# ilyakurdyukov/jpeg-quantsmooth

Hardware: AMD Instinct MI355X
Metric: 8x8 blocks/s at q=3 niter=3 (higher is better)
Workload: dtype f32

## Files before the change

### jpeg-quantsmooth_amd/csrc/qs_kernels.hip

```cpp
#include <hip/hip_runtime.h>
#include <stdint.h>
#include <stdlib.h>
#include "qs_device.h"
#include "qs_devfn.h"



__device__ __forceinline__ void wave_lds_sync() {
  __builtin_amdgcn_fence(__ATOMIC_RELEASE, "wavefront");
  __builtin_amdgcn_wave_barrier();
  __builtin_amdgcn_fence(__ATOMIC_ACQUIRE, "wavefront");
}

__device__ __forceinline__ uint32_t mulc(uint32_t a, int c) {
  return (uint32_t)__mul24((int)a, c);
}

__device__ __forceinline__ uint32_t lshl13_add(uint32_t x, uint32_t b) {
  uint32_t r;
  asm("v_lshl_add_u32 %0, %1, 13, %2" : "=v"(r) : "v"(x), "v"(b));
  return r;
}

__device__ __forceinline__ void idct8(uint32_t (&v)[8], uint32_t bias) {
  uint32_t z1, z2, z3, z4, z5, t0, t1, t2, t3, e0, e1, e2, e3;
  z2 = v[2]; z3 = v[6];
  z1 = mulc(z2 + z3, 4433);
  asm volatile("" : "+v"(z1));
  t2 = z1 - mulc(z3, 15137);
  t3 = z1 + mulc(z2, 6270);
  t0 = lshl13_add(v[0] + v[4], bias);
  t1 = lshl13_add(v[0] - v[4], bias);
  e0 = t0 + t3; e3 = t0 - t3; e1 = t1 + t2; e2 = t1 - t2;
  t0 = v[7]; t1 = v[5]; t2 = v[3]; t3 = v[1];
  z1 = t0 + t3; z2 = t1 + t2; z3 = t0 + t2; z4 = t1 + t3;
  z5 = mulc(z3 + z4, 9633);
  asm volatile("" : "+v"(z5));
  t0 = mulc(t0, 2446);  t1 = mulc(t1, 16819);
  t2 = mulc(t2, 25172); t3 = mulc(t3, 12299);
  z1 = mulc(z1, 7373);  z2 = mulc(z2, 20995);
  z3 = mulc(z3, 16069); z4 = mulc(z4, 3196);
  z3 = z5 - z3; z4 = z5 - z4;
  t0 += z3 - z1; t1 += z4 - z2; t2 += z3 - z2; t3 += z4 - z1;
  v[0] = e0 + t3; v[7] = e0 - t3;
  v[1] = e1 + t2; v[6] = e1 - t2;
  v[2] = e2 + t1; v[5] = e2 - t1;
  v[3] = e3 + t0; v[4] = e3 - t0;
}

__device__ __forceinline__ void idct_pass1(uint32_t (&ws)[64]) {
#pragma unroll
  for (int x = 0; x < 8; ++x) {
    uint32_t col[8];
#pragma unroll
    for (int j = 0; j < 8; ++j) col[j] = ws[j * 8 + x];
    idct8(col, 1024u);
#pragma unroll
    for (int j = 0; j < 8; ++j) ws[j * 8 + x] = (uint32_t)((int32_t)col[j] >> 11);
  }
}

__device__ __forceinline__ void idct_pass2_row(uint32_t (&row)[8], int (&out)[8]) {
  idct8(row, 257u << 17);
#pragma unroll
  for (int j = 0; j < 8; ++j) {
    int z = (int32_t)row[j];
    z = min(max(z, 0), (256 << 18) - 1);
    out[j] = z >> 18;
  }
}

#define QS_PIX_BITS 0x45000000u
__device__ __forceinline__ void idct_pass2_row_f(uint32_t (&row)[8], float (&out)[8]) {
  idct8(row, 257u << 17);
#pragma unroll
  for (int j = 0; j < 8; ++j) {
    int z = (int32_t)row[j];
    z = min(max(z, 0), (256 << 18) - 1);
    out[j] = __builtin_bit_cast(float, __builtin_amdgcn_alignbit(QS_PIX_BITS >> 14, (uint32_t)z, 18));
  }
}
__device__ __forceinline__ float pix_from_byte(uint32_t v, int n) {
  return __builtin_bit_cast(float, QS_PIX_BITS | ((v >> (8 * n)) & 0xffu));
}

__device__ __forceinline__ void
store_pixel_row(uint8_t* __restrict__ org, int pitch, int y, const int (&o)[8], int bx, int by, int wblk, int hblk,
                int rep_top, int rep_bot) {
  uint2 pk;
  pk.x = (uint32_t)o[0] | ((uint32_t)o[1] << 8) | ((uint32_t)o[2] << 16) | ((uint32_t)o[3] << 24);
  pk.y = (uint32_t)o[4] | ((uint32_t)o[5] << 8) | ((uint32_t)o[6] << 16) | ((uint32_t)o[7] << 24);
  uint8_t* rp = org + (size_t)y * pitch;
  *reinterpret_cast<uint2*>(rp) = pk;
  const bool top = (y == 0 && by == 0 && rep_top), bot = (y == 7 && by == hblk - 1 && rep_bot);
  if (bx == 0) {
    rp[-1] = (uint8_t)o[0];
    if (top) rp[-1 - pitch] = (uint8_t)o[0];
    if (bot) rp[-1 + pitch] = (uint8_t)o[0];
  }
  if (bx == wblk - 1) {
    rp[8] = (uint8_t)o[7];
    if (top) rp[8 - pitch] = (uint8_t)o[7];
    if (bot) rp[8 + pitch] = (uint8_t)o[7];
  }
  if (top) *reinterpret_cast<uint2*>(rp - pitch) = pk;
  if (bot) *reinterpret_cast<uint2*>(rp + pitch) = pk;
}

__device__ __forceinline__ void
idct_ws_to_plane(uint32_t (&ws)[64], uint8_t* __restrict__ plane, int wblk, int hblk, int pitch,
                 int rep_top, int rep_bot, int blk) {
  const int by = blk / wblk, bx = blk - by * wblk;
  idct_pass1(ws);
  uint8_t* org = plane + (size_t)(by * 8 + 1) * pitch + QS_APRON_X + bx * 8;
#pragma unroll
  for (int y = 0; y < 8; ++y) {
    uint32_t row[8]; int o[8];
#pragma unroll
    for (int j = 0; j < 8; ++j) row[j] = ws[y * 8 + j];
    idct_pass2_row(row, o);
    store_pixel_row(org, pitch, y, o, bx, by, wblk, hblk, rep_top, rep_bot);
  }
}

__device__ __forceinline__ void
idct_wave_to_plane(const QsConsts* __restrict__ cst, int16_t* __restrict__ coef,
                   uint8_t* __restrict__ plane, int wblk, int hblk, int pitch,
                   int first, int defer, int rep_top, int rep_bot, int* __restrict__ status, int base, uint32_t* lds) {
  const int lane = threadIdx.x & 63;
  const int nblk = wblk * hblk;
  const int nvec = min(64, nblk - base) * 8;
  uint4* gsrc = reinterpret_cast<uint4*>(coef) + (size_t)base * 8;
  uint4 v[8];
#pragma unroll
  for (int j = 0; j < 8; ++j) {
    const int idx = j * 64 + lane;
    v[j] = make_uint4(0, 0, 0, 0);
    if (idx < nvec) v[j] = gsrc[idx];
  }
  if (first) {
    int q[8], bad = 0;
    qs_load_qraw8(cst, lane & 7, q);
#pragma unroll
    for (int j = 0; j < 8; ++j) v[j] = qs_dequant8<true>(v[j], q, bad);
    if (!defer) {
#pragma unroll
      for (int j = 0; j < 8; ++j) {
        const int idx = j * 64 + lane;
        if (idx < nvec) gsrc[idx] = v[j];
      }
    }
    if (bad) atomicOr(status, 1);
  }
  {
    const int m0 = (lane & 7) * 4;
#pragma unroll
    for (int j = 0; j < 8; ++j) {
      uint32_t* dst = lds + m0 * QS_LDS_PITCH + (j * 8 + (lane >> 3));
      dst[0] = v[j].x; dst[QS_LDS_PITCH] = v[j].y; dst[2 * QS_LDS_PITCH] = v[j].z; dst[3 * QS_LDS_PITCH] = v[j].w;
    }
  }
  wave_lds_sync();
  const uint32_t* col = lds + lane;
  uint32_t ws[64];
#pragma unroll
  for (int r = 0; r < 32; ++r) {
    const uint32_t d = col[r * QS_LDS_PITCH];
    ws[r * 2] = (uint32_t)(int32_t)(int16_t)(d & 0xffff);
    ws[r * 2 + 1] = (uint32_t)((int32_t)d >> 16);
  }
  if (base + lane < nblk) idct_ws_to_plane(ws, plane, wblk, hblk, pitch, rep_top, rep_bot, base + lane);
}

__global__ void __launch_bounds__(256)
qs_idct_plane_kernel(const QsConsts* __restrict__ cst, int16_t* __restrict__ coef,
                     uint8_t* __restrict__ plane, int wblk, int hblk, int pitch,
                     int first, int rep_top, int rep_bot, int* __restrict__ status) {
  __shared__ uint32_t lds_all[4][32 * QS_LDS_PITCH];
  const int wave = threadIdx.x >> 6;
  const int base = __builtin_amdgcn_readfirstlane((int)(blockIdx.x * 256 + wave * 64));
  if (base >= wblk * hblk) return;
  idct_wave_to_plane(cst, coef, plane, wblk, hblk, pitch, first & 1, first & 2, rep_top, rep_bot, status, base, lds_all[wave]);
}

__global__ void __launch_bounds__(256)
qs_idct_set_kernel(const QsPlaneSet set, int first) {
  __shared__ uint32_t lds_all[4][32 * QS_LDS_PITCH];
  const int wave = threadIdx.x >> 6;
  const int w = __builtin_amdgcn_readfirstlane((int)(blockIdx.x * 4 + wave));
  if (w >= set.wave0[set.n]) return;
  const int i = qs_set_find(set, w);
  const QsPlaneRef& r = set.ref[i];
  const int base = (w - set.wave0[i]) * 64;
  if (base >= r.wblk * r.hblk) return;
  idct_wave_to_plane(r.cst, r.coef, r.plane, r.wblk, r.hblk, r.pitch, first, r.mode & QS_PLANE_QUANT,
                     r.mode & QS_PLANE_REP_TOP, r.mode & QS_PLANE_REP_BOT, r.status, base, lds_all[wave]);
}



typedef int16_t __attribute__((may_alias)) lds_i16;
__device__ __forceinline__ int lds_coef(const uint32_t* col, int i) {
  const lds_i16* p = reinterpret_cast<const lds_i16*>(col + (i >> 1) * QS_LDS_PITCH) + (i & 1);
  return *p;
}
__device__ __forceinline__ void lds_set_coef(uint32_t* col, int i, int v) {
  lds_i16* p = reinterpret_cast<lds_i16*>(col + (i >> 1) * QS_LDS_PITCH) + (i & 1);
  *p = (lds_i16)v;
}

static_assert(QS_LDS_PITCH * 4 == 260, "the literal offsets below assume a 260-byte row pitch");
#define QS_LDS16_GROUP(BASE, W, N0, O) \
  asm volatile("ds_read_i16 %0, %16 offset:" #O "\n\tds_read_i16 %1, %16 offset:" #O "+2\n\t" \
               "ds_read_i16 %2, %16 offset:" #O "+260\n\tds_read_i16 %3, %16 offset:" #O "+262\n\t" \
               "ds_read_i16 %4, %16 offset:" #O "+520\n\tds_read_i16 %5, %16 offset:" #O "+522\n\t" \
               "ds_read_i16 %6, %16 offset:" #O "+780\n\tds_read_i16 %7, %16 offset:" #O "+782\n\t" \
               "ds_read_i16 %8, %16 offset:" #O "+1040\n\tds_read_i16 %9, %16 offset:" #O "+1042\n\t" \
               "ds_read_i16 %10, %16 offset:" #O "+1300\n\tds_read_i16 %11, %16 offset:" #O "+1302\n\t" \
               "ds_read_i16 %12, %16 offset:" #O "+1560\n\tds_read_i16 %13, %16 offset:" #O "+1562\n\t" \
               "ds_read_i16 %14, %16 offset:" #O "+1820\n\tds_read_i16 %15, %16 offset:" #O "+1822\n\t" \
               "s_waitcnt lgkmcnt(0)" \
               : "=&v"(W[(N0) + 0]), "=&v"(W[(N0) + 1]), "=&v"(W[(N0) + 2]), "=&v"(W[(N0) + 3]), \
                 "=&v"(W[(N0) + 4]), "=&v"(W[(N0) + 5]), "=&v"(W[(N0) + 6]), "=&v"(W[(N0) + 7]), \
                 "=&v"(W[(N0) + 8]), "=&v"(W[(N0) + 9]), "=&v"(W[(N0) + 10]), "=&v"(W[(N0) + 11]), \
                 "=&v"(W[(N0) + 12]), "=&v"(W[(N0) + 13]), "=&v"(W[(N0) + 14]), "=&v"(W[(N0) + 15]) \
               : "v"(BASE) : "memory")
__device__ __forceinline__ void lds_read_block_i16(const uint32_t* col, uint32_t (&ws)[64]) {
  typedef const __attribute__((address_space(3))) uint32_t* lds_ptr;
  const uint32_t a0 = (uint32_t)(uintptr_t)(lds_ptr)col;
  const uint32_t a1 = a0 + 8 * 260, a2 = a0 + 16 * 260, a3 = a0 + 24 * 260;
  QS_LDS16_GROUP(a0, ws, 0, 0);
  QS_LDS16_GROUP(a1, ws, 16, 0);
  QS_LDS16_GROUP(a2, ws, 32, 0);
  QS_LDS16_GROUP(a3, ws, 48, 0);
}
__device__ __forceinline__ void lds_read_block_i16_1(const uint32_t* col, uint32_t (&ws)[64]) {
  typedef const __attribute__((address_space(3))) uint32_t* lds_ptr;
  const uint32_t a0 = (uint32_t)(uintptr_t)(lds_ptr)col;
  QS_LDS16_GROUP(a0, ws, 0, 0);
  QS_LDS16_GROUP(a0, ws, 16, 2080);
  QS_LDS16_GROUP(a0, ws, 32, 4160);
  QS_LDS16_GROUP(a0, ws, 48, 6240);
}

#define QS_PIX_SCALE 0.000244140625f
#define QS_TERM_D(D, W) { \
    float u_ = __builtin_amdgcn_fmed3f(Rs - __builtin_fabsf(D), 0.0f, 1.0f); \
    float t_ = u_ * u_; \
    float x_ = (D) * t_; \
    float y_ = (W) * t_; \
    num = num + x_ * y_; \
    den = den + y_ * y_; }
#define QS_TERM(A, B, W) { float d_ = (A) - (B); QS_TERM_D(d_, W) }

typedef float qs_w16 __attribute__((ext_vector_type(16)));
typedef int qs_i4 __attribute__((ext_vector_type(4)));
#define QS_SWAIT(BUF) asm volatile("s_waitcnt lgkmcnt(0)" : "+s"(BUF) : : "memory")

#define QS_WAVES_PER_WG 4
#define QS_SMOOTH_MIN_WAVES 3
#define QS_RESIDENT_WG (256 * QS_SMOOTH_MIN_WAVES * 4 / QS_WAVES_PER_WG)
#define QS_PRIO_SLOW 3
#define QS_PRIO_TERMS 0

#define QS_TERM_OPT(COND, A, B, W) { float d_, t_; \
        asm volatile( \
          "s_cmp_lg_u32 %[c], 0\n\t" \
          "s_cbranch_scc1 1f\n\t" \
          "v_sub_f32 %[d], %[a], %[b]\n\t" \
          "v_sub_f32 %[t], %[r], |%[d]| clamp\n\t" \
          "v_mul_f32 %[t], %[t], %[t]\n\t" \
          "v_mul_f32 %[d], %[d], %[t]\n\t" \
          "v_mul_f32 %[t], %[w], %[t]\n\t" \
          "v_mul_f32 %[d], %[d], %[t]\n\t" \
          "v_add_f32 %[n], %[n], %[d]\n\t" \
          "v_mul_f32 %[d], %[t], %[t]\n\t" \
          "v_add_f32 %[e], %[e], %[d]\n" \
          "1:" \
          : [n] "+v"(num), [e] "+v"(den), [d] "=&v"(d_), [t] "=&v"(t_) \
          : [a] "v"(A), [b] "v"(B), [w] "s"(W), [r] "s"(Rs), [c] "s"(COND) : "scc"); }
#define QS_TERM_ASM(A, B, W) { float d_, t_; \
        asm volatile( \
          "v_sub_f32 %[d], %[a], %[b]\n\t" \
          "v_sub_f32 %[t], %[r], |%[d]| clamp\n\t" \
          "v_mul_f32 %[t], %[t], %[t]\n\t" \
          "v_mul_f32 %[d], %[d], %[t]\n\t" \
          "v_mul_f32 %[t], %[w], %[t]\n\t" \
          "v_mul_f32 %[d], %[d], %[t]\n\t" \
          "v_add_f32 %[n], %[n], %[d]\n\t" \
          "v_mul_f32 %[d], %[t], %[t]\n\t" \
          "v_add_f32 %[e], %[e], %[d]" \
          : [n] "+v"(num), [e] "+v"(den), [d] "=&v"(d_), [t] "=&v"(t_) \
          : [a] "v"(A), [b] "v"(B), [w] "s"(W), [r] "s"(Rs)); }

#define QS_TERM_D_ASM(D, W) { float d_, t_; \
        asm volatile( \
          "v_sub_f32 %[t], %[r], |%[a]| clamp\n\t" \
          "v_mul_f32 %[t], %[t], %[t]\n\t" \
          "v_mul_f32 %[d], %[a], %[t]\n\t" \
          "v_mul_f32 %[t], %[w], %[t]\n\t" \
          "v_mul_f32 %[d], %[d], %[t]\n\t" \
          "v_add_f32 %[n], %[n], %[d]\n\t" \
          "v_mul_f32 %[d], %[t], %[t]\n\t" \
          "v_add_f32 %[e], %[e], %[d]" \
          : [n] "+v"(num), [e] "+v"(den), [d] "=&v"(d_), [t] "=&v"(t_) \
          : [a] "v"(D), [w] "s"(W), [r] "s"(Rs)); }
#ifndef QS_HOIST_DIAG
#define QS_HOIST_DIAG 32
#endif
#ifndef QS_Q1_SKIP
#define QS_Q1_SKIP 1
#endif
#ifndef QS_STASH
#define QS_STASH 1
#endif
#define QS_X_STASH 0
#define QS_X_EDGE 8
#define QS_X_REB 16
#define QS_X_DWORDS 20
static_assert(QS_WAVES_PER_WG * (32 * QS_LDS_PITCH + QS_X_DWORDS * 64) * 4 <= 160 * 1024 / 3, "LDS budget of three workgroups per CU");
typedef unsigned long long __attribute__((address_space(3))) qs_lds_u64;
__device__ __forceinline__ void qs_lds_add64(qs_lds_u64* p, long long v) {
  __hip_atomic_fetch_add(p, (unsigned long long)v, __ATOMIC_RELAXED, __HIP_MEMORY_SCOPE_WAVEFRONT);
}
__device__ __forceinline__ qs_lds_u64* qs_xreb(const uint32_t* col, const uint32_t* lds, int n) {
  typedef const __attribute__((address_space(3))) uint32_t* lds_ptr;
  uint32_t a = (uint32_t)(uintptr_t)(lds_ptr)col;
  asm volatile("" : "+v"(a));
  const uint32_t b = (uint32_t)(uintptr_t)(lds_ptr)lds;
  return (qs_lds_u64*)(a * 2u - b + (uint32_t)((32 * QS_LDS_PITCH + (QS_X_REB + 2 * n) * 64) * 4));
}

#define QS_SMOOTH_KERNEL_NAME qs_smooth_plane_kernel
#include "qs_smooth_kernel.inc"
#undef QS_SMOOTH_KERNEL_NAME
#define QS_SMOOTH_KERNEL_NAME qs_smooth_set_kernel
#define QS_SMOOTH_SET 1
#include "qs_smooth_kernel.inc"
#undef QS_SMOOTH_KERNEL_NAME
#undef QS_SMOOTH_SET

#define QS_DP_KERNEL_NAME qs_smooth_dp_kernel
#include "qs_smooth_dp_kernel.inc"
#undef QS_DP_KERNEL_NAME
#define QS_DP_KERNEL_NAME qs_smooth_dp_set_kernel
#define QS_DP_SET 1
#include "qs_smooth_dp_kernel.inc"
#undef QS_DP_KERNEL_NAME
#undef QS_DP_SET

__global__ void __launch_bounds__(256)
qs_clamp_kernel(int16_t* __restrict__ coef, size_t nvec) {
  size_t i = (size_t)blockIdx.x * 256 + threadIdx.x;
  const size_t stride = (size_t)gridDim.x * 256;
  uint4* p = reinterpret_cast<uint4*>(coef);
  for (; i < nvec; i += stride) {
    uint4 v = p[i];
    uint32_t d[4] = {v.x, v.y, v.z, v.w};
#pragma unroll
    for (int c = 0; c < 4; ++c) {
      int lo = (int16_t)(d[c] & 0xffff), hi = (int32_t)d[c] >> 16;
      lo = min(max(lo, -1023), 1023); hi = min(max(hi, -1023), 1023);
      d[c] = ((uint32_t)lo & 0xffffu) | ((uint32_t)hi << 16);
    }
    p[i] = make_uint4(d[0], d[1], d[2], d[3]);
  }
}

__global__ void __launch_bounds__(256)
qs_dequant_kernel(const QsConsts* __restrict__ cst, int16_t* __restrict__ coef, size_t nvec) {
  size_t i = (size_t)blockIdx.x * 256 + threadIdx.x;
  const size_t stride = (size_t)gridDim.x * 256;
  uint4* p = reinterpret_cast<uint4*>(coef);
  for (; i < nvec; i += stride) {
    uint4 v = p[i];
    uint32_t d[4] = {v.x, v.y, v.z, v.w};
    const int j = (int)(i & 7);
#pragma unroll
    for (int c = 0; c < 4; ++c) {
      int lo = (int16_t)(d[c] & 0xffff), hi = (int32_t)d[c] >> 16;
      lo *= cst->qraw[j * 8 + c * 2]; hi *= cst->qraw[j * 8 + c * 2 + 1];
      d[c] = ((uint32_t)lo & 0xffffu) | ((uint32_t)hi << 16);
    }
    p[i] = make_uint4(d[0], d[1], d[2], d[3]);
  }
}

#include "qs_launch.h"

void qs_launch_idct_plane(const QsConsts* cst, int16_t* coef, uint8_t* plane, int wblk, int hblk,
                          int first, int rep_top, int rep_bot, int* status, hipStream_t s) {
  const int nblk = wblk * hblk;
  const int f = first == 3 ? 3 : first ? 1 : 0;
  hipLaunchKernelGGL(qs_idct_plane_kernel, dim3((nblk + 255) / 256), dim3(256), 0, s,
                     cst, coef, plane, wblk, hblk, qs_plane_pitch(wblk), f, rep_top, rep_bot, status);
}

#define QS_DP_WAVES 4
static int qs_dp_waves(int groups) {
  static const int on = [] { const char* v = getenv("QS_HIP_DP"); return v ? atoi(v) : 1; }();
  static const int lim = [] { const char* v = getenv("QS_HIP_DP_GROUPS"); return v ? atoi(v) : 768; }();
  static const int lim2 = [] { const char* v = getenv("QS_HIP_DP_GROUPS2"); return v ? atoi(v) : 1536; }();
  if (!on) return 0;
  return groups <= lim ? QS_DP_WAVES : groups <= lim2 ? 2 : 0;
}

void qs_launch_smooth_plane(const QsConsts* cst, int16_t* coef, const uint8_t* plane, uint8_t* plane_next, int rep_top, int rep_bot,
                            int wblk, int hblk, int diag, int rebalance, int final_clamp, int blk_begin, int blk_end, hipStream_t s) {
  const int n = blk_end - blk_begin;
  if (n <= 0) return;
  const int pitch = qs_plane_pitch(wblk);
  const int rep = (rep_top ? QS_PLANE_REP_TOP : 0) | (rep_bot ? QS_PLANE_REP_BOT : 0);
  if (const int nw = qs_dp_waves((n + 63) / 64)) {
    const dim3 g((n + 63) / 64), b(64 * nw);
#define QS_GO_DP(D, W) hipLaunchKernelGGL((qs_smooth_dp_kernel<D, W>), g, b, 0, s, cst, coef, plane, plane_next, rep, wblk, hblk, pitch, rebalance, final_clamp, blk_begin, blk_end)
    if (nw == 2) { if (diag) QS_GO_DP(true, 2); else QS_GO_DP(false, 2); }
    else if (diag) QS_GO_DP(true, QS_DP_WAVES); else QS_GO_DP(false, QS_DP_WAVES);
#undef QS_GO_DP
    return;
  }
  const int per_wg = 64 * QS_WAVES_PER_WG;
  const dim3 grid((n + per_wg - 1) / per_wg), block(per_wg);
#define QS_GO(K) hipLaunchKernelGGL(K, grid, block, 0, s, cst, coef, plane, plane_next, rep, wblk, hblk, pitch, rebalance, final_clamp, blk_begin, blk_end)
  if (diag) QS_GO(qs_smooth_plane_kernel<true>); else QS_GO(qs_smooth_plane_kernel<false>);
#undef QS_GO
}

void qs_launch_idct_set(const QsPlaneSet& set, int first, hipStream_t s) {
  const int nw = set.wave0[set.n];
  if (nw <= 0) return;
  hipLaunchKernelGGL(qs_idct_set_kernel, dim3((nw + 3) / 4), dim3(256), 0, s, set, first);
}

void qs_launch_smooth_set(const QsPlaneSet& set, int diag, int final_clamp, hipStream_t s) {
  const int nw = set.wave0[set.n];
  if (nw <= 0) return;
  if (const int dw = qs_dp_waves(nw)) {
    const dim3 g(nw), b(64 * dw);
#define QS_GO_DP(D, W) hipLaunchKernelGGL((qs_smooth_dp_set_kernel<D, W>), g, b, 0, s, set, final_clamp)
    if (dw == 2) { if (diag) QS_GO_DP(true, 2); else QS_GO_DP(false, 2); }
    else if (diag) QS_GO_DP(true, QS_DP_WAVES); else QS_GO_DP(false, QS_DP_WAVES);
#undef QS_GO_DP
    return;
  }
  const dim3 grid((nw + QS_WAVES_PER_WG - 1) / QS_WAVES_PER_WG), block(64 * QS_WAVES_PER_WG);
  if (diag) hipLaunchKernelGGL(qs_smooth_set_kernel<true>, grid, block, 0, s, set, final_clamp);
  else      hipLaunchKernelGGL(qs_smooth_set_kernel<false>, grid, block, 0, s, set, final_clamp);
}

void qs_launch_clamp(int16_t* coef, size_t nblk, hipStream_t s) {
  const size_t nvec = nblk * 8;
  const int grid = (int)((nvec + 255) / 256 < 8192 ? (nvec + 255) / 256 : 8192);
  hipLaunchKernelGGL(qs_clamp_kernel, dim3(grid ? grid : 1), dim3(256), 0, s, coef, nvec);
}

void qs_launch_dequant(const QsConsts* cst, int16_t* coef, size_t nblk, hipStream_t s) {
  const size_t nvec = nblk * 8;
  const int grid = (int)((nvec + 255) / 256 < 8192 ? (nvec + 255) / 256 : 8192);
  hipLaunchKernelGGL(qs_dequant_kernel, dim3(grid ? grid : 1), dim3(256), 0, s, cst, coef, nvec);
}
```

### jpeg-quantsmooth_amd/csrc/qs_smooth_kernel.inc

```
template <bool DIAG>
__global__ void __launch_bounds__(64 * QS_WAVES_PER_WG, QS_SMOOTH_MIN_WAVES)
#ifdef QS_SMOOTH_SET
QS_SMOOTH_KERNEL_NAME(const QsPlaneSet set, int final_clamp) {
  __shared__ __attribute__((aligned(16))) uint32_t lds_all[QS_WAVES_PER_WG][32 * QS_LDS_PITCH + (DIAG ? 0 : QS_X_DWORDS * 64)];
#if QS_STASH
  __shared__ uint32_t stash_all[QS_WAVES_PER_WG][2 * 8 * 64];
#endif
  const int lane = threadIdx.x & 63, wave = DIAG ? (int)(threadIdx.x >> 6) : __builtin_amdgcn_readfirstlane((int)(threadIdx.x >> 6));
  uint32_t* lds = lds_all[wave];
  uint32_t* col = lds + lane;
  const int gw = __builtin_amdgcn_readfirstlane((int)(blockIdx.x * QS_WAVES_PER_WG + wave));
  if (gw >= set.wave0[set.n]) return;
  const int pi = qs_set_find(set, gw);
  const QsConsts* __restrict__ cst = set.ref[pi].cst;
  int16_t* __restrict__ coef = set.ref[pi].coef;
  const uint8_t* __restrict__ plane = set.ref[pi].plane;
  const int wblk = set.ref[pi].wblk, hblk = set.ref[pi].hblk, pitch = set.ref[pi].pitch;
  const int rebalance = set.ref[pi].mode & QS_PLANE_REBALANCE;
  const int nblk = wblk * hblk;
  const int base = (gw - set.wave0[pi]) * 64;
  (void)hblk;
#else
QS_SMOOTH_KERNEL_NAME(const QsConsts* __restrict__ cst, int16_t* __restrict__ coef,
                       const uint8_t* __restrict__ plane, uint8_t* __restrict__ plane_next, int rep,
                       int wblk, int hblk, int pitch,
                       int rebalance, int final_clamp, int blk_begin, int blk_end) {
  __shared__ __attribute__((aligned(16))) uint32_t lds_all[QS_WAVES_PER_WG][32 * QS_LDS_PITCH + (DIAG ? 0 : QS_X_DWORDS * 64)];
#if QS_STASH
  __shared__ uint32_t stash_all[QS_WAVES_PER_WG][2 * 8 * 64];
#endif
  const int lane = threadIdx.x & 63, wave = DIAG ? (int)(threadIdx.x >> 6) : __builtin_amdgcn_readfirstlane((int)(threadIdx.x >> 6));
  uint32_t* lds = lds_all[wave];
  uint32_t* col = lds + lane;
  const int nblk = blk_end;
  const int base = blk_begin + (blockIdx.x * QS_WAVES_PER_WG + wave) * 64;
#endif
  if (base >= nblk) return;
  const int tail_prio = __builtin_amdgcn_readfirstlane(
      (gridDim.x > QS_RESIDENT_WG && blockIdx.x >= (gridDim.x / QS_RESIDENT_WG) * QS_RESIDENT_WG) ? 1 : 0);
  const int nvec = min(64, nblk - base) * 8;
#ifdef QS_STAGGER
  { unsigned hwid; asm volatile("s_getreg_b32 %0, hwreg(HW_REG_HW_ID)" : "=s"(hwid)); if (hwid & 1u) __builtin_amdgcn_s_sleep(QS_STAGGER); }
#endif

  uint4* gsrc = reinterpret_cast<uint4*>(coef) + (size_t)base * 8;
  uint32_t bigacc = 0;
#define QS_BIG_ACC(V) if constexpr (!DIAG) bigacc |= ((V).x ^ ((V).x << 1)) | ((V).y ^ ((V).y << 1)) | ((V).z ^ ((V).z << 1)) | ((V).w ^ ((V).w << 1))
#ifdef QS_SMOOTH_SET
  if (set.ref[pi].mode & QS_PLANE_QUANT) {
    const int m0 = (lane & 7) * 4;
    int q[8], unused = 0;
    qs_load_qraw8(cst, lane & 7, q);
#pragma unroll
    for (int j = 0; j < 8; ++j) {
      const int idx = j * 64 + lane;
      uint4 v = make_uint4(0, 0, 0, 0);
      if (idx < nvec) v = gsrc[idx];
      v = qs_dequant8<false>(v, q, unused);
      QS_BIG_ACC(v);
      uint32_t* dst = lds + m0 * QS_LDS_PITCH + (j * 8 + (lane >> 3));
      dst[0] = v.x; dst[QS_LDS_PITCH] = v.y; dst[2 * QS_LDS_PITCH] = v.z; dst[3 * QS_LDS_PITCH] = v.w;
    }
  } else
#endif
  {
    const int m0 = (lane & 7) * 4;
#pragma unroll
    for (int j = 0; j < 8; ++j) {
      const int idx = j * 64 + lane;
      uint4 v = make_uint4(0, 0, 0, 0);
      if (idx < nvec) v = gsrc[idx];
      QS_BIG_ACC(v);
      uint32_t* dst = lds + m0 * QS_LDS_PITCH + (j * 8 + (lane >> 3));
      dst[0] = v.x; dst[QS_LDS_PITCH] = v.y; dst[2 * QS_LDS_PITCH] = v.z; dst[3 * QS_LDS_PITCH] = v.w;
    }
  }

  const int blk = min(base + lane, nblk - 1);
  const int by = blk / wblk, bx = blk - by * wblk;
  const uint8_t* org = plane + (size_t)(by * 8 + 1) * pitch + QS_APRON_X + bx * 8;
  uint32_t edge[8];
  {
    const uint2 t = *reinterpret_cast<const uint2*>(org - pitch);
    const uint2 b = *reinterpret_cast<const uint2*>(org + (size_t)8 * pitch);
    edge[0] = t.x; edge[1] = t.y; edge[2] = b.x; edge[3] = b.y;
    uint32_t l[8], r[8];
#pragma unroll
    for (int y = 0; y < 8; ++y) {
      l[y] = org[(ptrdiff_t)y * pitch - 1];
      r[y] = org[(ptrdiff_t)y * pitch + 8];
    }
    edge[4] = l[0] | (l[1] << 8) | (l[2] << 16) | (l[3] << 24);
    edge[5] = l[4] | (l[5] << 8) | (l[6] << 16) | (l[7] << 24);
    edge[6] = r[0] | (r[1] << 8) | (r[2] << 16) | (r[3] << 24);
    edge[7] = r[4] | (r[5] << 8) | (r[6] << 16) | (r[7] << 24);
  }
  uint32_t* const xcol = col + 32 * QS_LDS_PITCH;
  if constexpr (!DIAG) {
#pragma unroll
    for (int e = 0; e < 8; ++e) xcol[(QS_X_EDGE + e) * 64] = edge[e];
    *qs_xreb(col, lds, 0) = 0; *qs_xreb(col, lds, 1) = 0;
  }
  wave_lds_sync();

  constexpr int TS = DIAG ? 272 : 160;
  float px[DIAG ? 64 : 1];
  float bd[32];
  constexpr int NH = DIAG ? QS_HOIST_DIAG : 1;
  float hd[NH];
  float dh[DIAG ? 1 : 56], dv[DIAG ? 1 : 56];

  int kfirst = 63;
#if QS_STASH
  int stash_hi = 0;
#endif
  uint32_t chg = 0;
  uint64_t chg_any = 0;
#undef QS_BIG_ACC
  const bool big_wave = !DIAG && __builtin_amdgcn_ballot_w64((bigacc & 0xC000C000u) != 0) != 0;
  long long reb_m0 = 0, reb_m1 = 0;
  const float* tabp = cst->tab;
  const int32_t* recp = &cst->rec[0][0];
  qs_w16 WA, WB;
  qs_i4 REC;
  qs_i4 RECN;
  asm volatile("s_load_dwordx4 %0, %2, %3\n\ts_load_dwordx16 %1, %4, %5\n\ts_waitcnt lgkmcnt(0)"
               : "=&s"(REC), "=&s"(WA) : "s"(recp), "s"(63u * 16u), "s"(tabp), "s"((uint32_t)63 * (TS * 4)) : "memory");
  RECN = REC;

#pragma unroll 1
  for (int g = 0; g < 14; ++g) {
    __builtin_amdgcn_s_setprio(QS_PRIO_SLOW);
    if (g == 0 || (DIAG ? __builtin_amdgcn_ballot_w64(chg != 0) != 0 : chg_any != 0)) {
      chg = 0;
      chg_any = 0;
      uint32_t ws[64];
      if constexpr (DIAG) lds_read_block_i16(col, ws); else lds_read_block_i16_1(col, ws);
#if QS_STASH
      {
        uint32_t* stash = DIAG ? stash_all[wave] + lane : xcol + QS_X_STASH * 64;
#pragma unroll
        for (int x = 0; x < 8; ++x) {
          uint32_t c[8];
          const bool low = x <= (DIAG ? 1 : 0), high = x >= (DIAG ? 6 : 7);
          const int slot = (x == 0 || x == 7) ? 0 : 1;
          bool reuse = false, store = false;
          if (low) { reuse = g >= 1 && g <= 7 - x; store = g == 0; }
          if (high) {
            const int fin = 15 - x;
            const bool have = (stash_hi >> (x - 6)) & 1;
            reuse = g >= fin && have; store = g >= fin && !have;
          }
          if ((low || high) && reuse) {
#pragma unroll
            for (int j = 0; j < 8; ++j) c[j] = stash[(slot * 8 + j) * 64];
          } else {
#pragma unroll
            for (int j = 0; j < 8; ++j) c[j] = ws[j * 8 + x];
            idct8(c, 1024u);
#pragma unroll
            for (int j = 0; j < 8; ++j) c[j] = (uint32_t)((int32_t)c[j] >> 11);
            if ((low || high) && store) {
#pragma unroll
              for (int j = 0; j < 8; ++j) stash[(slot * 8 + j) * 64] = c[j];
              if (high) stash_hi |= 1 << (x - 6);
            }
          }
#pragma unroll
          for (int j = 0; j < 8; ++j) ws[j * 8 + x] = c[j];
        }
      }
#else
      idct_pass1(ws);
#endif
      if constexpr (!DIAG) {
        float prev[8];
#pragma unroll
        for (int y = 0; y < 8; ++y) {
          uint32_t row[8]; float o[8];
#pragma unroll
          for (int j = 0; j < 8; ++j) row[j] = ws[y * 8 + j];
          idct_pass2_row_f(row, o);
#pragma unroll
          for (int x = 0; x < 7; ++x) dh[y * 7 + x] = o[x] - o[x + 1];
          if (y > 0) {
#pragma unroll
            for (int x = 0; x < 8; ++x) dv[(y - 1) * 8 + x] = prev[x] - o[x];
          }
          if (y == 0 || y == 7) {
            const uint32_t e0 = xcol[(QS_X_EDGE + (y ? 2 : 0)) * 64], e1 = xcol[(QS_X_EDGE + (y ? 3 : 1)) * 64];
#pragma unroll
            for (int x = 0; x < 8; ++x) bd[(y ? 8 : 0) + x] = o[x] - pix_from_byte(x < 4 ? e0 : e1, x & 3);
          }
          {
            const uint32_t el = xcol[(QS_X_EDGE + 4 + (y >> 2)) * 64], er = xcol[(QS_X_EDGE + 6 + (y >> 2)) * 64];
            bd[16 + y] = o[0] - pix_from_byte(el, y & 3);
            bd[24 + y] = o[7] - pix_from_byte(er, y & 3);
          }
#pragma unroll
          for (int x = 0; x < 8; ++x) prev[x] = o[x];
          __builtin_amdgcn_sched_barrier(0);
        }
      } else {
#pragma unroll
      for (int y = 0; y < 8; ++y) {
        uint32_t row[8]; float o[8];
#pragma unroll
        for (int j = 0; j < 8; ++j) row[j] = ws[y * 8 + j];
        idct_pass2_row_f(row, o);
#pragma unroll
        for (int j = 0; j < 8; ++j) px[y * 8 + j] = o[j];
      }
#pragma unroll
      for (int e = 0; e < 8; ++e) asm volatile("" : "+v"(edge[e]));
#pragma unroll
      for (int x = 0; x < 8; ++x) {
        bd[x]      = px[x]         - pix_from_byte(edge[0 + (x >> 2)], x & 3);
        bd[8 + x]  = px[56 + x]    - pix_from_byte(edge[2 + (x >> 2)], x & 3);
        bd[16 + x] = px[x * 8]     - pix_from_byte(edge[4 + (x >> 2)], x & 3);
        bd[24 + x] = px[x * 8 + 7] - pix_from_byte(edge[6 + (x >> 2)], x & 3);
      }
#pragma unroll
      for (int t = 0; t < NH; ++t) hd[t] = px[(t / 7) * 8 + t % 7] - px[(t / 7) * 8 + t % 7 + 1];
      }
    }
    const int len = min(g + 1, 15 - g);
    const int klast = max(kfirst - len + 1, 1);
#pragma unroll 1
    for (int k = kfirst; k >= klast; --k) {
      if constexpr (DIAG) {
#pragma unroll
        for (int p = 0; p < 64; ++p) asm volatile("" : "+v"(px[p]));
      }
      const int md = REC[3];
      const int x2k = (REC[0] >> 16) & 31, qk = REC[1] & 0xffff, x1k = REC[1] >> 16;
      const uint32_t lds_off = ((uint32_t)md >> QS_REC_LDS_SHIFT) & 0x3fffu;
      int rs_bits = REC[2];
      asm volatile("" : "+s"(rs_bits));
      const float Rs = __builtin_bit_cast(float, rs_bits);
      const uint32_t kb = (uint32_t)k * (TS * 4);
      const uint32_t kb_nxt = kb - (uint32_t)(TS * 4);
      const uint32_t kb_s = (uint32_t)__builtin_amdgcn_readfirstlane((int)kb);
      const uint32_t kb_nxt_s = (uint32_t)__builtin_amdgcn_readfirstlane((int)kb_nxt);
      const uint32_t next_first = kb_nxt + (((uint32_t)md >> QS_REC_NXT_SHIFT) & 0x100u);
      const uint32_t after_V = DIAG ? kb + 640u : next_first;
      const uint32_t after_B = (md & QS_REC_V_ANY) ? kb + 384u : after_V;
#if QS_Q1_SKIP
      if (__builtin_expect(md & QS_REC_Q1, 0)) {
        {
          const int c0 = *reinterpret_cast<lds_i16*>(reinterpret_cast<char*>(col) + lds_off);
          if constexpr (DIAG) {
            reb_m0 += (long long)(c0 * c0);
            reb_m1 += (long long)(c0 * c0);
          } else {
            qs_lds_u64* const xreb = qs_xreb(col, lds, 0);
            qs_lds_add64(xreb, (long long)(c0 * c0));
            qs_lds_add64(xreb + 64, (long long)(c0 * c0));
          }
        }
        asm volatile("s_load_dwordx16 %0, %2, %3\n\ts_load_dwordx4 %1, %4, %5\n\ts_waitcnt lgkmcnt(0)"
                     : "=&s"(WA), "=&s"(RECN)
                     : "s"(tabp), "s"((uint32_t)__builtin_amdgcn_readfirstlane((int)next_first)), "s"(recp),
                       "s"((uint32_t)(k - 1) * 16u) : "memory");
        REC = RECN;
      } else
#endif
      {
      float num = 0.0f, den = 0.0f;
      asm volatile("s_setprio %c1\n\ts_cmp_eq_u32 %0, 0\n\ts_cbranch_scc1 1f\n\ts_setprio %c2\n1:"
                   : : "s"(tail_prio), "i"(QS_PRIO_TERMS), "i"(QS_PRIO_TERMS + 1) : "scc");

#define QS_ROW_D(W, Y) { \
        _Pragma("unroll") for (int x = 0; x < 7; ++x) { \
          QS_TERM(px[(Y) * 8 + x], px[(Y) * 8 + x + 9], W[x]) \
          QS_TERM(px[(Y) * 8 + x + 1], px[(Y) * 8 + x + 8], W[8 + x]) } }
#define QS_EDGE16(W, J0) { \
        _Pragma("unroll") for (int j = 0; j < 16; ++j) { \
          if constexpr (DIAG) QS_TERM_D(bd[(J0) + j], W[j]) \
          else QS_TERM_D_ASM(bd[(J0) + j], W[j]) } }
#define QS_HOISTED_TERM(T, WT) else if ((T) < NH) QS_TERM_D_ASM(hd[(T) % NH], WT)
#define QS_ROWS_H_M(W, Y0, MODE) { \
        _Pragma("unroll") for (int yy = 0; yy < 2; ++yy) \
        _Pragma("unroll") for (int x = 0; x < 7; ++x) { \
          if (((MODE) == 2 && (x & 1)) || ((MODE) == 1 && x == 3)) {} \
          else if constexpr (!DIAG) QS_TERM_D_ASM(dh[((Y0) + yy) * 7 + x], W[yy * 8 + x]) \
          QS_HOISTED_TERM(((Y0) + yy) * 7 + x, W[yy * 8 + x]) \
          else QS_TERM_ASM(px[((Y0) + yy) * 8 + x], px[((Y0) + yy) * 8 + x + 1], W[yy * 8 + x]) } }
#define QS_ROWS_V_M(W, Y0, NY, MODE) { \
        _Pragma("unroll") for (int yy = 0; yy < (NY); ++yy) \
        _Pragma("unroll") for (int x = 0; x < 8; ++x) { \
          if (((MODE) == 2 && (((Y0) + yy) & 1)) || ((MODE) == 1 && (Y0) + yy == 3)) {} \
          else if constexpr (!DIAG) QS_TERM_D_ASM(dv[((Y0) + yy) * 8 + x], W[yy * 8 + x]) \
          else QS_TERM_ASM(px[((Y0) + yy) * 8 + x], px[((Y0) + yy) * 8 + x + 8], W[yy * 8 + x]) } }

      const uint32_t rec_next = (uint32_t)(k - 1) * 16u;
#define QS_ISSUE(NXT, BYTEOFF) \
      asm volatile("s_load_dwordx16 %0, %3, %4" : "=&s"(NXT), "+v"(num), "+v"(den) \
                   : "s"(tabp), "s"((uint32_t)__builtin_amdgcn_readfirstlane((int)(BYTEOFF))) : "memory")
#define QS_ISSUE_K(NXT, IMM) \
      asm volatile("s_load_dwordx16 %0, %3, %4 offset:%c5" : "=&s"(NXT), "+v"(num), "+v"(den) \
                   : "s"(tabp), "s"(kb_s), "i"(IMM) : "memory")
#define QS_LAND(NXT) asm volatile("s_waitcnt lgkmcnt(0)" : "+s"(NXT), "+v"(num), "+v"(den) : : "memory")
#define QS_ISSUE_R(NXT, BYTEOFF) \
      asm volatile("s_load_dwordx16 %0, %4, %5\n\ts_load_dwordx4 %1, %6, %7" : "=&s"(NXT), "=&s"(RECN), "+v"(num), "+v"(den) \
                   : "s"(tabp), "s"((uint32_t)__builtin_amdgcn_readfirstlane((int)(BYTEOFF))), "s"(recp), "s"(rec_next) : "memory")
#define QS_LAND_R(NXT) asm volatile("s_waitcnt lgkmcnt(0)" : "+s"(NXT), "+s"(RECN), "+v"(num), "+v"(den) : : "memory")
#define QS_T4(O) "s_load_dword %1, %4, %5 offset:" #O "\n\ts_load_dword %1, %4, %5 offset:" #O "+0x40\n\ts_load_dword %1, %4, %5 offset:" #O "+0x80\n\ts_load_dword %1, %4, %5 offset:" #O "+0xc0\n\t"
#define QS_ISSUE_T(NXT, IMM) \
      uint32_t touch; \
      if (DIAG) asm volatile("s_load_dwordx16 %0, %4, %6 offset:%c7\n\t" QS_T4(0x0) QS_T4(0x100) QS_T4(0x200) QS_T4(0x300) "s_load_dword %1, %4, %5 offset:0x400" \
                   : "=&s"(NXT), "=&s"(touch), "+v"(num), "+v"(den) \
                   : "s"(tabp), "s"(kb_nxt_s), "s"(kb_s), "i"(IMM) : "memory"); \
      else      asm volatile("s_load_dwordx16 %0, %4, %6 offset:%c7\n\t" QS_T4(0x0) QS_T4(0x100) "s_load_dword %1, %4, %5 offset:0x200\n\ts_load_dword %1, %4, %5 offset:0x240" \
                   : "=&s"(NXT), "=&s"(touch), "+v"(num), "+v"(den) \
                   : "s"(tabp), "s"(kb_nxt_s), "s"(kb_s), "i"(IMM) : "memory")
#define QS_LAND_T(NXT) asm volatile("s_waitcnt lgkmcnt(0)" : "+s"(NXT), "+s"(touch), "+v"(num), "+v"(den) : : "memory")
#define QS_H_SECTION(MODE) { \
        QS_ISSUE_K(WB, 64);  QS_ROWS_H_M(WA, 0, MODE) QS_LAND(WB); \
        QS_ISSUE_K(WA, 128); QS_ROWS_H_M(WB, 2, MODE) QS_LAND(WA); \
        QS_ISSUE_K(WB, 192); QS_ROWS_H_M(WA, 4, MODE) QS_LAND(WB); \
        QS_ISSUE_K(WA, 256); QS_ROWS_H_M(WB, 6, MODE) QS_LAND(WA); }
      if (md & QS_REC_H_ANY) {
        if (md & QS_REC_H_SKIP4) QS_H_SECTION(2)
        else if (md & QS_REC_H_EVEN) QS_H_SECTION(1)
        else QS_H_SECTION(0)
      }
      QS_ISSUE_T(WB, 320); QS_EDGE16(WA, 0) QS_LAND_T(WB);
      if (!DIAG && !(md & QS_REC_V_ANY)) { QS_ISSUE_R(WA, after_B); QS_EDGE16(WB, 16) QS_LAND_R(WA); }
      else                   { QS_ISSUE(WA, after_B);   QS_EDGE16(WB, 16) QS_LAND(WA); }
#define QS_V_SECTION(MODE) { \
        QS_ISSUE_K(WB, 448); QS_ROWS_V_M(WA, 0, 2, MODE) QS_LAND(WB); \
        QS_ISSUE_K(WA, 512); QS_ROWS_V_M(WB, 2, 2, MODE) QS_LAND(WA); \
        QS_ISSUE_K(WB, 576); QS_ROWS_V_M(WA, 4, 2, MODE) QS_LAND(WB); \
        if (!DIAG) { QS_ISSUE_R(WA, after_V); QS_ROWS_V_M(WB, 6, 1, MODE) QS_LAND_R(WA); } \
        else       { QS_ISSUE(WA, after_V);   QS_ROWS_V_M(WB, 6, 1, MODE) QS_LAND(WA); } }
      if (md & QS_REC_V_ANY) {
        if (md & QS_REC_V_SKIP4) QS_V_SECTION(2)
        else if (md & QS_REC_V_EVEN) QS_V_SECTION(1)
        else QS_V_SECTION(0)
      }
      if (DIAG) {
        QS_ISSUE_K(WB, 704);  QS_ROW_D(WA, 0) QS_LAND(WB);
        QS_ISSUE_K(WA, 768);  QS_ROW_D(WB, 1) QS_LAND(WA);
        QS_ISSUE_K(WB, 832);  QS_ROW_D(WA, 2) QS_LAND(WB);
        QS_ISSUE_K(WA, 896);  QS_ROW_D(WB, 3) QS_LAND(WA);
        QS_ISSUE_K(WB, 960);  QS_ROW_D(WA, 4) QS_LAND(WB);
        QS_ISSUE_K(WA, 1024); QS_ROW_D(WB, 5) QS_LAND(WA);
        QS_ISSUE_R(WB, next_first); QS_ROW_D(WA, 6) QS_LAND_R(WB);
        WA = WB;
      }
#undef QS_ROWS_H_M
#undef QS_HOISTED_TERM
#undef QS_ROWS_V_M
#undef QS_H_SECTION
#undef QS_V_SECTION
#undef QS_ISSUE
#undef QS_ISSUE_K
#undef QS_LAND
#undef QS_ISSUE_R
#undef QS_LAND_R
#undef QS_ISSUE_T
#undef QS_LAND_T
#undef QS_T4

      __builtin_amdgcn_s_setprio(QS_PRIO_SLOW);
      lds_i16* const cptr = reinterpret_cast<lds_i16*>(reinterpret_cast<char*>(col) + lds_off);
      const int c0 = *cptr;
      const int r = f2i_x86(round_half_away((num / den) * 4096.0f));
      {
        int orig, lo, hi;
        interval(c0, qk, x1k, x2k, orig, lo, hi);
        int v = (int)((uint32_t)c0 - (uint32_t)r);
        v = min(max(v, lo), hi);
        if constexpr (DIAG) {
          *cptr = (lds_i16)v;
          chg |= (uint32_t)(v ^ c0);
          if (rebalance) {
            reb_m0 += (long long)(v * orig);
            reb_m1 += (long long)(orig * orig);
          }
        } else {
          if (__builtin_expect(big_wave, 0)) { asm volatile("" : "+v"(v)); v = r ? v : c0; }
          *cptr = (lds_i16)v;
          chg_any |= __builtin_amdgcn_ballot_w64(v != c0);
          if (rebalance) {
            qs_lds_u64* const xreb = qs_xreb(col, lds, 0);
            qs_lds_add64(xreb, (long long)(v * orig));
            qs_lds_add64(xreb + 64, (long long)(orig * orig));
          }
        }
      }
      REC = RECN;
      }
    }
    kfirst = klast - 1;
  }
  QS_SWAIT(WA);

  if (rebalance) {
    long long m0 = DIAG ? reb_m0 : (long long)*qs_xreb(col, lds, 0), m1 = DIAG ? reb_m1 : (long long)*qs_xreb(col, lds, 1);
    const bool big = big_wave;
    if (big) {
      m0 = 0; m1 = 0;
#pragma unroll 1
      for (int n = 1; n < 64; ++n) {
        const int c = lds_coef(col, n);
        int orig, lo, hi;
        interval(c, cst->qn[n], cst->x1n[n], cst->x2n[n], orig, lo, hi);
        m0 += (long long)(c * orig);
        m1 += (long long)(orig * orig);
      }
    }
    if (m1 > m0) {
      const int mul = (int)(((m1 << 13) + (m0 >> 1)) / m0);
#pragma unroll 9
      for (int n = 1; n < 64; ++n) {
        const int c = lds_coef(col, n);
        int orig, lo, hi;
        interval(c, cst->qn[n], cst->x1n[n], cst->x2n[n], orig, lo, hi);
        if (big) {
          const int div = cst->qn[n], a = (int16_t)orig;
          hi = a + (a < 0 ? div >> 1 : (div - 1) >> 1);
          lo = a - (a > 0 ? div >> 1 : (div - 1) >> 1);
        }
        int v = (c * mul + 0x1000) >> 13;
        v = min(max(v, lo), hi);
        lds_set_coef(col, n, v);
      }
    }
  }
  wave_lds_sync();

  {
    int lane2 = DIAG ? lane : (int)__builtin_amdgcn_mbcnt_hi(~0u, __builtin_amdgcn_mbcnt_lo(~0u, 0u));
    asm volatile("" : "+v"(lane2));
    const int lane = lane2;
    const int m0 = (lane & 7) * 4;
#pragma unroll
    for (int j = 0; j < 8; ++j) {
      const int idx = j * 64 + lane;
      const uint32_t* s = lds + m0 * QS_LDS_PITCH + (j * 8 + (lane >> 3));
      uint32_t d[4] = {s[0], s[QS_LDS_PITCH], s[2 * QS_LDS_PITCH], s[3 * QS_LDS_PITCH]};
      if (final_clamp) {
#pragma unroll
        for (int c = 0; c < 4; ++c) {
          int lo = (int16_t)(d[c] & 0xffff), hi = (int32_t)d[c] >> 16;
          lo = min(max(lo, -1023), 1023); hi = min(max(hi, -1023), 1023);
          d[c] = ((uint32_t)lo & 0xffffu) | ((uint32_t)hi << 16);
        }
      }
      if (idx < nvec) gsrc[idx] = make_uint4(d[0], d[1], d[2], d[3]);
    }
  }

#ifdef QS_SMOOTH_SET
  int pi2 = pi;
  asm volatile("" : "+s"(pi2));
  uint8_t* __restrict__ plane_next = set.ref[pi2].plane_next;
  const int rep = set.ref[pi2].mode, wblk2 = set.ref[pi2].wblk, hblk2 = set.ref[pi2].hblk, pitch2 = set.ref[pi2].pitch;
#else
  const int wblk2 = wblk, hblk2 = hblk, pitch2 = pitch;
#endif
  if (plane_next) {
    uint32_t ws[64];
    if constexpr (DIAG) lds_read_block_i16(col, ws); else lds_read_block_i16_1(col, ws);
    int lane3 = DIAG ? lane : (int)__builtin_amdgcn_mbcnt_hi(~0u, __builtin_amdgcn_mbcnt_lo(~0u, 0u));
    if constexpr (!DIAG) asm volatile("" : "+v"(lane3));
    if (base + lane3 < nblk)
      idct_ws_to_plane(ws, plane_next, wblk2, hblk2, pitch2, rep & QS_PLANE_REP_TOP, rep & QS_PLANE_REP_BOT, base + lane3);
  }
}

#undef QS_ROW_D
#undef QS_EDGE16
```

Baseline: 281.8 million.

## Stash luma idct columns as 16-bit and keep rebalance sums in registers

```diff
diff --git a/jpeg-quantsmooth_amd/csrc/qs_kernels.hip b/jpeg-quantsmooth_amd/csrc/qs_kernels.hip
--- a/jpeg-quantsmooth_amd/csrc/qs_kernels.hip
+++ b/jpeg-quantsmooth_amd/csrc/qs_kernels.hip
@@ -3,6 +3,7 @@
 #include <stdlib.h>
 #include "qs_device.h"
 #include "qs_devfn.h"
+#include "qs_stash16.h"
 
 
 
@@ -316,19 +317,73 @@
 #endif
 #define QS_X_STASH 0
 #define QS_X_EDGE 8
-#define QS_X_REB 16
+#define QS_X_STASH_C 16
 #define QS_X_DWORDS 20
 static_assert(QS_WAVES_PER_WG * (32 * QS_LDS_PITCH + QS_X_DWORDS * 64) * 4 <= 160 * 1024 / 3, "LDS budget of three workgroups per CU");
-typedef unsigned long long __attribute__((address_space(3))) qs_lds_u64;
-__device__ __forceinline__ void qs_lds_add64(qs_lds_u64* p, long long v) {
-  __hip_atomic_fetch_add(p, (unsigned long long)v, __ATOMIC_RELAXED, __HIP_MEMORY_SCOPE_WAVEFRONT);
-}
-__device__ __forceinline__ qs_lds_u64* qs_xreb(const uint32_t* col, const uint32_t* lds, int n) {
+static_assert(32 * QS_LDS_PITCH * 4 + QS_X_STASH * 256 == 8320 && QS_X_STASH_C == 16, "the literal offsets below");
+#define QS_ST16_OFFS(SLOT) \
+  "i"(8320 + qs_stash16_byte(SLOT, 0)), "i"(8320 + qs_stash16_byte(SLOT, 1)), "i"(8320 + qs_stash16_byte(SLOT, 2)), \
+  "i"(8320 + qs_stash16_byte(SLOT, 3)), "i"(8320 + qs_stash16_byte(SLOT, 4)), "i"(8320 + qs_stash16_byte(SLOT, 5)), \
+  "i"(8320 + qs_stash16_byte(SLOT, 6)), "i"(8320 + qs_stash16_byte(SLOT, 7))
+template <int SLOT>
+__device__ __forceinline__ void qs_stash16_read(const uint32_t* col, uint32_t (&c)[8]) {
   typedef const __attribute__((address_space(3))) uint32_t* lds_ptr;
-  uint32_t a = (uint32_t)(uintptr_t)(lds_ptr)col;
-  asm volatile("" : "+v"(a));
-  const uint32_t b = (uint32_t)(uintptr_t)(lds_ptr)lds;
-  return (qs_lds_u64*)(a * 2u - b + (uint32_t)((32 * QS_LDS_PITCH + (QS_X_REB + 2 * n) * 64) * 4));
+  const uint32_t a = (uint32_t)(uintptr_t)(lds_ptr)col;
+  asm volatile("ds_read_i16 %0, %8 offset:%c9\n\tds_read_i16 %1, %8 offset:%c10\n\t"
+               "ds_read_i16 %2, %8 offset:%c11\n\tds_read_i16 %3, %8 offset:%c12\n\t"
+               "ds_read_i16 %4, %8 offset:%c13\n\tds_read_i16 %5, %8 offset:%c14\n\t"
+               "ds_read_i16 %6, %8 offset:%c15\n\tds_read_i16 %7, %8 offset:%c16\n\t"
+               "s_waitcnt lgkmcnt(0)"
+               : "=&v"(c[0]), "=&v"(c[1]), "=&v"(c[2]), "=&v"(c[3]), "=&v"(c[4]), "=&v"(c[5]), "=&v"(c[6]), "=&v"(c[7])
+               : "v"(a), QS_ST16_OFFS(SLOT) : "memory");
+}
+template <int SLOT>
+__device__ __forceinline__ void qs_stash16_write(const uint32_t* col, const uint32_t (&c)[8]) {
+  typedef const __attribute__((address_space(3))) uint32_t* lds_ptr;
+  const uint32_t a = (uint32_t)(uintptr_t)(lds_ptr)col;
+  asm volatile("ds_write_b16 %8, %0 offset:%c9\n\tds_write_b16 %8, %1 offset:%c10\n\t"
+               "ds_write_b16 %8, %2 offset:%c11\n\tds_write_b16 %8, %3 offset:%c12\n\t"
+               "ds_write_b16 %8, %4 offset:%c13\n\tds_write_b16 %8, %5 offset:%c14\n\t"
+               "ds_write_b16 %8, %6 offset:%c15\n\tds_write_b16 %8, %7 offset:%c16\n\t"
+               "s_waitcnt lgkmcnt(0)"
+               : : "v"(c[0]), "v"(c[1]), "v"(c[2]), "v"(c[3]), "v"(c[4]), "v"(c[5]), "v"(c[6]), "v"(c[7]),
+                   "v"(a), QS_ST16_OFFS(SLOT) : "memory");
+}
+#ifndef QS_LUMA_SLOTS
+#define QS_LUMA_SLOTS 2
+#endif
+static_assert(QS_LUMA_SLOTS >= 1 && QS_LUMA_SLOTS <= QS_ST16_SLOTS, "stash slots of the luma walk");
+template <int X>
+__device__ __forceinline__ void qs_luma_pass1_col(uint32_t (&ws)[64], const uint32_t* col, int g, int& stash_hi) {
+  constexpr bool low = X < QS_LUMA_SLOTS, high = X > 7 - QS_LUMA_SLOTS;
+  constexpr int slot = low ? X : 7 - X, bit = low ? 4 + slot : slot;
+  uint32_t c[8];
+  bool reuse = false, store = false;
+  if constexpr (low) { reuse = g >= 1 && g <= qs_stash16_low_last(slot) && ((stash_hi >> bit) & 1); store = g == 0; }
+  if constexpr (high) {
+    const bool have = (stash_hi >> bit) & 1;
+    reuse = g >= qs_stash16_high_first(slot) && have; store = g >= qs_stash16_high_first(slot) && !have;
+  }
+  if (reuse) {
+    if constexpr (low || high) qs_stash16_read<slot>(col, c);
+  } else {
+#pragma unroll
+    for (int j = 0; j < 8; ++j) c[j] = ws[j * 8 + X];
+    idct8(c, 1024u);
+#pragma unroll
+    for (int j = 0; j < 8; ++j) c[j] = (uint32_t)((int32_t)c[j] >> 11);
+    if constexpr (low || high) {
+      if (store) {
+        const int32_t ci[8] = {(int32_t)c[0], (int32_t)c[1], (int32_t)c[2], (int32_t)c[3], (int32_t)c[4], (int32_t)c[5], (int32_t)c[6], (int32_t)c[7]};
+        if (__builtin_amdgcn_ballot_w64(!qs_stash16_fits(ci)) == 0) {
+          qs_stash16_write<slot>(col, c);
+          stash_hi |= 1 << bit;
+        }
+      }
+    }
+  }
+#pragma unroll
+  for (int j = 0; j < 8; ++j) ws[j * 8 + X] = c[j];
 }
 
 #define QS_SMOOTH_KERNEL_NAME qs_smooth_plane_kernel
diff --git a/jpeg-quantsmooth_amd/csrc/qs_smooth_kernel.inc b/jpeg-quantsmooth_amd/csrc/qs_smooth_kernel.inc
--- a/jpeg-quantsmooth_amd/csrc/qs_smooth_kernel.inc
+++ b/jpeg-quantsmooth_amd/csrc/qs_smooth_kernel.inc
@@ -99,7 +99,6 @@
   if constexpr (!DIAG) {
 #pragma unroll
     for (int e = 0; e < 8; ++e) xcol[(QS_X_EDGE + e) * 64] = edge[e];
-    *qs_xreb(col, lds, 0) = 0; *qs_xreb(col, lds, 1) = 0;
   }
   wave_lds_sync();
 
@@ -117,8 +116,10 @@
   uint32_t chg = 0;
   uint64_t chg_any = 0;
 #undef QS_BIG_ACC
-  const bool big_wave = !DIAG && __builtin_amdgcn_ballot_w64((bigacc & 0xC000C000u) != 0) != 0;
+  const bool big_wave = !DIAG && __builtin_amdgcn_ballot_w64((bigacc & QS_BIG_PAIR_MASK) != 0) != 0;
+  const bool wide_wave = !DIAG && __builtin_amdgcn_ballot_w64((bigacc & QS_WIDE_PAIR_MASK) != 0) != 0;
   long long reb_m0 = 0, reb_m1 = 0;
+  uint32_t reb32_m0 = 0, reb32_m1 = 0;
   const float* tabp = cst->tab;
   const int32_t* recp = &cst->rec[0][0];
   qs_w16 WA, WB;
@@ -137,12 +138,17 @@
       uint32_t ws[64];
       if constexpr (DIAG) lds_read_block_i16(col, ws); else lds_read_block_i16_1(col, ws);
 #if QS_STASH
-      {
-        uint32_t* stash = DIAG ? stash_all[wave] + lane : xcol + QS_X_STASH * 64;
+      if constexpr (!DIAG) {
+        qs_luma_pass1_col<0>(ws, col, g, stash_hi); qs_luma_pass1_col<1>(ws, col, g, stash_hi);
+        qs_luma_pass1_col<2>(ws, col, g, stash_hi); qs_luma_pass1_col<3>(ws, col, g, stash_hi);
+        qs_luma_pass1_col<4>(ws, col, g, stash_hi); qs_luma_pass1_col<5>(ws, col, g, stash_hi);
+        qs_luma_pass1_col<6>(ws, col, g, stash_hi); qs_luma_pass1_col<7>(ws, col, g, stash_hi);
+      } else {
+        uint32_t* stash = stash_all[wave] + lane;
 #pragma unroll
         for (int x = 0; x < 8; ++x) {
           uint32_t c[8];
-          const bool low = x <= (DIAG ? 1 : 0), high = x >= (DIAG ? 6 : 7);
+          const bool low = x <= 1, high = x >= 6;
           const int slot = (x == 0 || x == 7) ? 0 : 1;
           bool reuse = false, store = false;
           if (low) { reuse = g >= 1 && g <= 7 - x; store = g == 0; }
@@ -253,9 +259,8 @@
             reb_m0 += (long long)(c0 * c0);
             reb_m1 += (long long)(c0 * c0);
           } else {
-            qs_lds_u64* const xreb = qs_xreb(col, lds, 0);
-            qs_lds_add64(xreb, (long long)(c0 * c0));
-            qs_lds_add64(xreb + 64, (long long)(c0 * c0));
+            reb32_m0 = qs_reb32_add(reb32_m0, c0, c0);
+            reb32_m1 = qs_reb32_add(reb32_m1, c0, c0);
           }
         }
         asm volatile("s_load_dwordx16 %0, %2, %3\n\ts_load_dwordx4 %1, %4, %5\n\ts_waitcnt lgkmcnt(0)"
@@ -384,9 +389,8 @@
           *cptr = (lds_i16)v;
           chg_any |= __builtin_amdgcn_ballot_w64(v != c0);
           if (rebalance) {
-            qs_lds_u64* const xreb = qs_xreb(col, lds, 0);
-            qs_lds_add64(xreb, (long long)(v * orig));
-            qs_lds_add64(xreb + 64, (long long)(orig * orig));
+            reb32_m0 = qs_reb32_add(reb32_m0, v, orig);
+            reb32_m1 = qs_reb32_add(reb32_m1, orig, orig);
           }
         }
       }
@@ -398,9 +402,9 @@
   QS_SWAIT(WA);
 
   if (rebalance) {
-    long long m0 = DIAG ? reb_m0 : (long long)*qs_xreb(col, lds, 0), m1 = DIAG ? reb_m1 : (long long)*qs_xreb(col, lds, 1);
+    long long m0 = DIAG ? reb_m0 : (long long)reb32_m0, m1 = DIAG ? reb_m1 : (long long)reb32_m1;
     const bool big = big_wave;
-    if (big) {
+    if (wide_wave) {
       m0 = 0; m1 = 0;
 #pragma unroll 1
       for (int n = 1; n < 64; ++n) {
diff --git a/jpeg-quantsmooth_amd/csrc/qs_stash16.h b/jpeg-quantsmooth_amd/csrc/qs_stash16.h
--- /dev/null
+++ b/jpeg-quantsmooth_amd/csrc/qs_stash16.h
@@ -0,0 +1,52 @@
+#ifndef QS_STASH16_H
+#define QS_STASH16_H
+#include <stdint.h>
+
+#if defined(__HIPCC__) || defined(__CUDACC__)
+#define QS_ST16_HD __host__ __device__ __forceinline__
+#else
+#define QS_ST16_HD static inline
+#endif
+
+QS_ST16_HD int32_t qs_st16_max3(int32_t a, int32_t b, int32_t c) { int32_t m = a > b ? a : b; return m > c ? m : c; }
+QS_ST16_HD int32_t qs_st16_min3(int32_t a, int32_t b, int32_t c) { int32_t m = a < b ? a : b; return m < c ? m : c; }
+QS_ST16_HD bool qs_stash16_fits(const int32_t (&c)[8]) {
+  int32_t hi = qs_st16_max3(c[0], c[1], c[2]), lo = qs_st16_min3(c[0], c[1], c[2]);
+  hi = qs_st16_max3(hi, c[3], c[4]); lo = qs_st16_min3(lo, c[3], c[4]);
+  hi = qs_st16_max3(hi, c[5], c[6]); lo = qs_st16_min3(lo, c[5], c[6]);
+  hi = hi > c[7] ? hi : c[7];        lo = lo < c[7] ? lo : c[7];
+  return hi <= 32767 && lo >= -32768;
+}
+QS_ST16_HD uint16_t qs_stash16_park(int32_t v) { return (uint16_t)((uint32_t)v & 0xffffu); }
+QS_ST16_HD int32_t qs_stash16_fetch(uint16_t h) { return (int32_t)(int16_t)h; }
+
+#define QS_ST16_SLOTS 3
+QS_ST16_HD constexpr int qs_stash16_byte(int slot, int j) {
+  return slot < 2 ? j * 256 + slot * 2 : (16 + (j >> 1)) * 256 + (j & 1) * 2;
+}
+QS_ST16_HD constexpr int qs_stash16_low_last(int slot) { return 7 - slot; }
+QS_ST16_HD constexpr int qs_stash16_high_first(int slot) { return 8 + slot; }
+
+#define QS_REB32_LOG2 12
+#define QS_REB32_LIMIT (1 << QS_REB32_LOG2)
+#define QS_REB32_QMAX 0x800
+QS_ST16_HD constexpr uint64_t qs_reb32_bound() {
+  return 63ull * (uint64_t)(QS_REB32_LIMIT + QS_REB32_QMAX / 2) * (uint64_t)(QS_REB32_LIMIT + QS_REB32_QMAX);
+}
+static_assert(qs_reb32_bound() < (1ull << 32), "the 32-bit rebalance sums must hold the largest sums a narrow wave can form");
+static_assert(QS_REB32_LIMIT > 2048 + QS_REB32_QMAX / 2, "no wave of a job may be wide");
+static_assert(QS_REB32_LIMIT + QS_REB32_QMAX < (1 << 23), "operands of the 24-bit multiply");
+QS_ST16_HD constexpr uint32_t qs_pair_mask(int log2) { return (0xffffu & ~((2u << log2) - 1u)) * 0x10001u; }
+#define QS_BIG_PAIR_MASK qs_pair_mask(13)
+#define QS_WIDE_PAIR_MASK qs_pair_mask(QS_REB32_LOG2)
+static_assert(qs_pair_mask(13) == 0xC000C000u && qs_pair_mask(12) == 0xE000E000u, "pair masks");
+QS_ST16_HD uint32_t qs_pair_spread(uint32_t pair) { return pair ^ (pair << 1); }
+QS_ST16_HD uint32_t qs_reb32_add(uint32_t sum, int32_t a, int32_t b) {
+#if defined(__HIP_DEVICE_COMPILE__)
+  return sum + (uint32_t)__mul24(a, b);
+#else
+  return sum + (uint32_t)a * (uint32_t)b;
+#endif
+}
+
+#endif
```

New measurement: 282.8 million, median of 6. About the same (+0.4%).
